# hiroyasuakada/EgoRear

Measured on AMD Instinct MI355X. Metric: 4-view frames/sec (heatmap+MVFEx+3D lift), higher is better.
Workload: dtype f32 (fp16x2 split, 22-bit operands, fp32 accumulate)

## Files before the change

### egorear_amd/csrc/egr_stem_pool.h

```cpp
#pragma once
#include "egr_common.h"

template <int NW>
struct StemPool {
    f32x2 P0[8];
    f32x2 P1[8];
    f32x2 e0, e1;
    float amx = 0.f;

    static __device__ __forceinline__ int pc(int q, int half) { return (q & 1) + 4 * (q >> 1) + 2 * half; }

    __device__ __forceinline__ void reduce(const f32x16 (&acc)[2][2], const float (&sc)[2], const float (&sh)[2], int half) {
#pragma unroll
        for (int j = 0; j < 2; ++j) {
            float vm[16], v1[16];
#pragma unroll
            for (int r = 0; r < 16; ++r) {
                float t0 = acc[0][j][r] * sc[j] + sh[j], t1 = acc[1][j][r] * sc[j] + sh[j];
                t0 = t0 > 0.f ? t0 : 0.f;
                t1 = t1 > 0.f ? t1 : 0.f;
                v1[r] = t1;
                vm[r] = fmaxf(t0, t1);
                amx = fmaxf(amx, vm[r]);
            }
            float om[4], o1[4];
#pragma unroll
            for (int g = 0; g < 4; ++g) { om[g] = __shfl_xor(vm[4 * g + 3], 32); o1[g] = __shfl_xor(v1[4 * g + 3], 32); }
#pragma unroll
            for (int q = 0; q < 8; ++q) {
                const int g = q >> 1;
                float x0 = fmaxf(vm[2 * q], vm[2 * q + 1]), x1 = fmaxf(v1[2 * q], v1[2 * q + 1]);
                if (q & 1) { x0 = fmaxf(x0, vm[2 * q - 1]); x1 = fmaxf(x1, v1[2 * q - 1]); }
                else {
                    const float lm = half ? om[g] : (g > 0 ? om[g - 1] : 0.f), l1 = half ? o1[g] : (g > 0 ? o1[g - 1] : 0.f);
                    x0 = fmaxf(x0, lm); x1 = fmaxf(x1, l1);
                }
                P0[q][j] = x0; P1[q][j] = x1;
            }
            e0[j] = vm[15]; e1[j] = v1[15];
        }
    }

    static constexpr int XFLOATS = (NW - 1) * 16 * 64;

    __device__ __forceinline__ void publish(float* s_x, int wave, int l31, int half) const {
        if (wave < NW - 1) {
#pragma unroll
            for (int q = 0; q < 8; ++q) *reinterpret_cast<f32x2*>(&s_x[(wave * 16 + pc(q, half)) * 64 + 2 * l31]) = P1[q];
        }
    }

    static __device__ __forceinline__ void amax2(float* p, f32x2 v) {
        atomicMax(reinterpret_cast<int*>(p), __float_as_int(v[0]));
        atomicMax(reinterpret_cast<int*>(p) + 1, __float_as_int(v[1]));
    }

    __device__ __forceinline__ void finish(const float* s_x, int wave, int l31, int half, float* y, int n, int oy0, int ox0, int pho, int pwo) {
        if (wave > 0) {
#pragma unroll
            for (int q = 0; q < 8; ++q) {
                const f32x2 u = *reinterpret_cast<const f32x2*>(&s_x[((wave - 1) * 16 + pc(q, half)) * 64 + 2 * l31]);
                P0[q][0] = fmaxf(P0[q][0], u[0]); P0[q][1] = fmaxf(P0[q][1], u[1]);
            }
        }
        const int gp = (oy0 >> 1) + wave, gc0 = ox0 >> 1;
        float* const yrow = y + (((int64_t)n * pho + gp) * pwo + gc0) * 64 + 2 * l31;
        const bool arow = wave == 0 && oy0 > 0;
#pragma unroll
        for (int q = 0; q < 8; ++q) {
            float* const p = yrow + pc(q, half) * 64;
            if (arow || (q == 0 && half == 0 && ox0 > 0)) amax2(p, P0[q]);
            else *reinterpret_cast<f32x2*>(p) = P0[q];
        }
        if (half && gc0 + 16 < pwo) {
            amax2(yrow + 16 * 64, e0);
            if (gp + 1 < pho) amax2(yrow + (int64_t)pwo * 64 + 16 * 64, e1);
        }
        if (wave == NW - 1 && gp + 1 < pho) {
#pragma unroll
            for (int q = 0; q < 8; ++q) amax2(yrow + (int64_t)pwo * 64 + pc(q, half) * 64, P1[q]);
        }
    }
};

template <int NW>
__global__ __launch_bounds__(256) void stem_pool_init_kernel(float* y, int images, int pho, int pwo) {
    const int rows = pho / NW - ((pho % NW) ? 0 : 1), cols = pwo / 16 - ((pwo % 16) ? 0 : 1);
    const int64_t na = (int64_t)images * rows * pwo * 16, nb = (int64_t)images * pho * cols * 16;
    int64_t i = (int64_t)blockIdx.x * 256 + threadIdx.x;
    int n, p, c;
    if (i < na) {
        const int q = (int)(i & 15);
        int64_t t = i >> 4;
        c = (int)(t % pwo); t /= pwo;
        p = ((int)(t % rows) + 1) * NW; n = (int)(t / rows);
        i = q;
    } else if (i < na + nb) {
        i -= na;
        const int q = (int)(i & 15);
        int64_t t = i >> 4;
        c = ((int)(t % cols) + 1) * 16; t /= cols;
        p = (int)(t % pho); n = (int)(t / pho);
        i = q;
    } else return;
    const f32x4 z = {0.f, 0.f, 0.f, 0.f};
    *reinterpret_cast<f32x4*>(y + (((int64_t)n * pho + p) * pwo + c) * 64 + i * 4) = z;
}

template <int NW>
static inline void stem_pool_init(float* y, int64_t images, int pho, int pwo, hipStream_t s) {
    const int rows = pho / NW - ((pho % NW) ? 0 : 1), cols = pwo / 16 - ((pwo % 16) ? 0 : 1);
    const int64_t total = images * ((int64_t)rows * pwo + (int64_t)pho * cols) * 16;
    if (total <= 0) return;
    hipLaunchKernelGGL(stem_pool_init_kernel<NW>, dim3((unsigned)((total + 255) / 256)), dim3(256), 0, s, y, (int)images, pho, pwo);
}
```

### egorear_amd/csrc/egr_stem_x6.hip

```cpp
#include "egr_common.h"
#include "egr_stem_pool.h"

namespace {

typedef __bf16 bf16x8 __attribute__((ext_vector_type(8)));
typedef _Float16 f16x8 __attribute__((ext_vector_type(8)));
typedef unsigned u32x4 __attribute__((ext_vector_type(4)));

constexpr int NW = 8, NT = NW * 64;
constexpr int TH = 2 * NW, TW = 32;
constexpr int PH = 2 * TH + 5;
constexpr int PW = 2 * TW + 5;
constexpr int PWS = 72;
constexpr int PATCH = 3 * PH * PWS;
constexpr int PLOADS = (PATCH + NT - 1) / NT;
constexpr int PPAIRS = (PATCH / 2 + NT - 1) / NT;
static_assert(PATCH % 2 == 0 && PWS % 2 == 0, "pixel pairs");
#ifndef STEM_PRESPLIT
#define STEM_PRESPLIT 1
#endif
#ifndef STEM_KS
#define STEM_KS 11
#endif
constexpr int KS = STEM_KS;
constexpr int WBYTES = KS * 2 * 3 * 1024;
constexpr int WBYTES2 = KS * 2 * 2 * 1024;

static_assert(StemPool<NW>::XFLOATS <= PATCH, "the pooling exchange area lives in a dead patch buffer");

__device__ __forceinline__ unsigned cvt_pk_bf16(float lo, float hi) {
    unsigned r;
    asm("v_cvt_pk_bf16_f32 %0, %1, %2" : "=v"(r) : "v"(lo), "v"(hi));
    return r;
}
__device__ __forceinline__ float bf16_hi_f32(unsigned p) { return __uint_as_float(p & 0xffff0000u); }
__device__ __forceinline__ float bf16_lo_f32(unsigned p) { return __uint_as_float(p << 16); }
__device__ __forceinline__ void split2_f16(float v0, float v1, float s, unsigned& h, unsigned& l) {
    asm("v_fma_mixlo_f16 %0, %1, %2, 0" : "=v"(h) : "v"(v0), "v"(s));
    asm("v_fma_mixhi_f16 %0, %1, %2, 0" : "+v"(h) : "v"(v1), "v"(s));
    asm("v_fma_mixlo_f16 %0, %1, %2, -%3 op_sel_hi:[0,0,1]" : "=v"(l) : "v"(v0), "v"(s), "v"(h));
    asm("v_fma_mixhi_f16 %0, %1, %2, -%3 op_sel:[0,0,1] op_sel_hi:[0,0,1]" : "+v"(l) : "v"(v1), "v"(s), "v"(h));
}
__device__ __forceinline__ void pow2_prescale(unsigned bits, float& s, float& inv) {
    int k = 141 - (int)(bits >> 23);
    k = k > 60 ? 60 : (k < -60 ? -60 : k);
    s = __uint_as_float((unsigned)(127 + k) << 23);
    inv = __uint_as_float((unsigned)(127 - k) << 23);
}

struct StemX6Args {
    const float* x;
    egr_nmap xmap;
    int n, h, w, ho, wo;
    const uint8_t* w6;
    const float* wds;
    const float* scale;
    const float* shift;
    float* y;
    int tiles_x, tiles_y;
    int64_t gx;
    unsigned* amax_out;
};

template <int PH_>
__device__ __forceinline__ constexpr int pair_off_t(int p) {
    const int pp = p > 20 ? 20 : p;
    return (pp / 7) * PH_ * PWS + (pp % 7) * PWS;
}

template <bool POOL, int NPL>
__global__ __launch_bounds__(NT, 1) void stem_x6_kernel(const StemX6Args a) {
    auto pair_off = [](int p) constexpr { return pair_off_t<PH>(p); };
    constexpr int WB = NPL == 3 ? WBYTES : WBYTES2, NPR = NPL == 3 ? 6 : 3;
    constexpr bool PRE = NPL == 2 && STEM_PRESPLIT;
    __shared__ __attribute__((aligned(16))) float s_patch[2][PATCH];
    __shared__ __attribute__((aligned(16))) uint8_t s_w[WB];
    __shared__ unsigned s_pmax[2][NW];
    const int tid = threadIdx.x, lane = tid & 63, wave = tid >> 6;
    const int l31 = lane & 31, half = lane >> 5;
    const int grp = blockIdx.y;
    const int tpi = a.tiles_x * a.tiles_y;
    const int total = a.n * tpi;
    const float* xg = a.x + grp * a.gx;
    const bool raw = a.scale == nullptr;
    float* y = a.y + (int64_t)grp * a.n * (POOL ? (a.ho >> 1) * (a.wo >> 1) : a.ho * a.wo) * 64;

    int p_lds[PLOADS], p_ci[PLOADS], p_py[PLOADS], p_px[PLOADS];
#pragma unroll
    for (int u = 0; u < PLOADS; ++u) {
        const int i = tid + NT * u;
        const int ci = i / (PH * PWS);
        const int r = i - ci * PH * PWS;
        p_ci[u] = ci; p_py[u] = r / PWS; p_px[u] = r - p_py[u] * PWS;
        p_lds[u] = (i < PATCH) ? i : -1;
    }
    auto fetch = [&](int tile, float (&v)[PLOADS]) {
        const int n = tile / tpi;
        const int t = tile - n * tpi;
        const int ty = t / a.tiles_x, tx = t - ty * a.tiles_x;
        const int iy0 = 2 * ty * TH - 3, ix0 = 2 * tx * TW - 3;
        const float* img = xg + egr_map(a.xmap, n);
#pragma unroll
        for (int u = 0; u < PLOADS; ++u) {
            const int iy = iy0 + p_py[u], ix = ix0 + p_px[u];
            const bool ok = p_lds[u] >= 0 && p_px[u] < PW && iy >= 0 && iy < a.h && ix >= 0 && ix < a.w;
            v[u] = ok ? img[((int64_t)p_ci[u] * a.h + iy) * a.w + ix] : 0.f;
        }
    };
    auto park = [&](int buf, const float (&v)[PLOADS]) {
        float m = 0.f;
#pragma unroll
        for (int u = 0; u < PLOADS; ++u)
            if (p_lds[u] >= 0) {
                s_patch[buf][p_lds[u]] = v[u];
                m = fmaxf(m, fabsf(v[u]));
            }
        if constexpr (NPL == 2) {
            m = wave_max(m);
            if (lane == 0) s_pmax[buf][wave] = __float_as_uint(m);
        }
    };
    int q_geo[PRE ? PPAIRS : 1];
    if constexpr (PRE) {
#pragma unroll
        for (int u = 0; u < PPAIRS; ++u) {
            const int i = 2 * (tid + NT * u);
            const int ci = i / (PH * PWS);
            const int r = i - ci * PH * PWS;
            const int py = r / PWS;
            q_geo[u] = (i < PATCH) ? ((ci << 16) | (py << 8) | (r - py * PWS)) : -1;
        }
    }
    auto fetch2 = [&](int tile, float (&v)[2 * PPAIRS]) {
        const int n = tile / tpi;
        const int t = tile - n * tpi;
        const int ty = t / a.tiles_x, tx = t - ty * a.tiles_x;
        const int iy0 = 2 * ty * TH - 3, ix0 = 2 * tx * TW - 3;
        const float* img = xg + egr_map(a.xmap, n);
#pragma unroll
        for (int u = 0; u < (PRE ? PPAIRS : 1); ++u) {
            const int g = q_geo[u], q_ci = g >> 16, q_py = (g >> 8) & 255, q_px = g & 255;
            const int iy = iy0 + q_py, ix = ix0 + q_px;
            const bool rowok = g >= 0 && iy >= 0 && iy < a.h;
            const float* rp = img + ((int64_t)q_ci * a.h + iy) * a.w + ix;
            v[2 * u] = (rowok && q_px < PW && ix >= 0 && ix < a.w) ? rp[0] : 0.f;
            v[2 * u + 1] = (rowok && q_px + 1 < PW && ix + 1 >= 0 && ix + 1 < a.w) ? rp[1] : 0.f;
        }
    };
    auto publish_max = [&](int buf, const float (&v)[2 * PPAIRS]) {
        float m = 0.f;
#pragma unroll
        for (int u = 0; u < 2 * PPAIRS; ++u) m = fmaxf(m, fabsf(v[u]));
        m = wave_max(m);
        if (lane == 0) s_pmax[buf][wave] = __float_as_uint(m);
    };
    auto park2 = [&](int buf, const float (&v)[2 * PPAIRS], float psc_) {
        unsigned* const ph = reinterpret_cast<unsigned*>(s_patch[buf]);
#pragma unroll
        for (int u = 0; u < (PRE ? PPAIRS : 1); ++u)
            if (q_geo[u] >= 0) {
                unsigned h, l;
                split2_f16(v[2 * u], v[2 * u + 1], psc_, h, l);
                ph[tid + NT * u] = h;
                ph[PATCH / 2 + tid + NT * u] = l;
            }
    };
    auto patch_scale = [&](int buf, float& s, float& inv) {
        unsigned m = s_pmax[buf][lane & (NW - 1)];
#pragma unroll
        for (int o = NW / 2; o > 0; o >>= 1) {
            const unsigned other = (unsigned)__shfl_xor((int)m, o, 64);
            m = other > m ? other : m;
        }
        pow2_prescale(__builtin_amdgcn_readfirstlane(m), s, inv);
    };

    {
        const u32x4* src = reinterpret_cast<const u32x4*>(a.w6 + (int64_t)grp * WB);
        for (int i = tid; i < WB / 16; i += NT) reinterpret_cast<u32x4*>(s_w)[i] = src[i];
    }
    float pv[PRE ? 1 : PLOADS];
    float pv2[PRE ? 2 * PPAIRS : 1];
    float psc = 1.f, pinv = 1.f;
    int tile = blockIdx.x;
    if constexpr (PRE) {
        if (tile < total) {
            fetch2(tile, pv2);
            publish_max(0, pv2);
        }
        __syncthreads();
        if (tile < total) {
            patch_scale(0, psc, pinv);
            park2(0, pv2, psc);
        }
    } else {
        if (tile < total) {
            fetch(tile, pv);
            park(0, pv);
        }
    }
    __syncthreads();

    const int abase0 = (2 * (2 * wave)) * PWS + 2 * l31;
    const int abase1 = (2 * (2 * wave + 1)) * PWS + 2 * l31;
    float sc[2], sh[2];
#pragma unroll
    for (int j = 0; j < 2; ++j) {
        sc[j] = raw ? 1.f : a.scale[grp * 64 + 2 * l31 + j];
        sh[j] = raw ? 0.f : a.shift[grp * 64 + 2 * l31 + j];
    }
    float wds[2] = {1.f, 1.f};
    if constexpr (NPL == 2) {
        wds[0] = a.wds[grp * 64 + 2 * l31];
        wds[1] = a.wds[grp * 64 + 2 * l31 + 1];
    }

    int buf = 0;
    float amx = 0.f;
    for (; tile < total; tile += gridDim.x, buf ^= 1) {
        const int next = tile + gridDim.x;
        if (next < total) {
            if constexpr (PRE) fetch2(next, pv2);
            else fetch(next, pv);
        }
        const float* sp = s_patch[buf];
        if constexpr (NPL == 2 && !PRE) patch_scale(buf, psc, pinv);
        const float pinv_cur = pinv;
        f32x16 acc[2][2];
#pragma unroll
        for (int i = 0; i < 2; ++i)
#pragma unroll
            for (int j = 0; j < 2; ++j)
#pragma unroll
                for (int r = 0; r < 16; ++r) acc[i][j][r] = 0.f;

        f32x2 raw_a[2][4];
        u32x4 sa[2][2][NPL];
        u32x4 bfr[2][2][NPL];
        auto read_a_pre = [&](int s, int par) {
            const int ao = half ? pair_off(2 * s + 1) : pair_off(2 * s);
            const unsigned* const ph = reinterpret_cast<const unsigned*>(sp);
            const unsigned* h0 = ph + ((abase0 + ao) >> 1);
            const unsigned* h1 = ph + ((abase1 + ao) >> 1);
#pragma unroll
            for (int e = 0; e < 4; ++e) {
                sa[par][0][0][e] = h0[e];
                sa[par][0][1][e] = h0[PATCH / 2 + e];
                sa[par][1][0][e] = h1[e];
                sa[par][1][1][e] = h1[PATCH / 2 + e];
            }
        };
        auto read_a = [&](int s) {
            const int ao = half ? pair_off(2 * s + 1) : pair_off(2 * s);
            const float* q0 = sp + abase0 + ao;
            const float* q1 = sp + abase1 + ao;
#pragma unroll
            for (int e = 0; e < 4; ++e) {
                raw_a[0][e] = *reinterpret_cast<const f32x2*>(q0 + 2 * e);
                raw_a[1][e] = *reinterpret_cast<const f32x2*>(q1 + 2 * e);
            }
        };
        auto read_b = [&](int s, int par) {
#pragma unroll
            for (int j = 0; j < 2; ++j)
#pragma unroll
                for (int pl = 0; pl < NPL; ++pl)
                    bfr[par][j][pl] = *reinterpret_cast<const u32x4*>(s_w + ((s * 2 + j) * NPL + pl) * 1024 + lane * 16);
        };
        auto split_pair = [&](int par, int i, int e) {
            const float v0 = raw_a[i][e][0], v1 = raw_a[i][e][1];
            if constexpr (NPL == 3) {
                const unsigned h = cvt_pk_bf16(v0, v1);
                const float r0 = v0 - bf16_lo_f32(h), r1 = v1 - bf16_hi_f32(h);
                const unsigned m = cvt_pk_bf16(r0, r1);
                sa[par][i][0][e] = h;
                sa[par][i][1][e] = m;
                sa[par][i][2][e] = cvt_pk_bf16(r0 - bf16_lo_f32(m), r1 - bf16_hi_f32(m));
            } else {
                unsigned h, l;
                split2_f16(v0, v1, psc, h, l);
                sa[par][i][0][e] = h;
                sa[par][i][1][e] = l;
            }
        };
        if constexpr (PRE) {
            read_a_pre(0, 0);
        } else {
            read_a(0);
        }
        read_b(0, 0);
        if constexpr (!PRE) {
#pragma unroll
            for (int c = 0; c < 8; ++c) split_pair(0, c >> 2, c & 3);
        }
#pragma unroll
        for (int s = 0; s < KS; ++s) {
            const int par = s & 1;
            if (s + 1 < KS) {
                if constexpr (PRE) read_a_pre(s + 1, par ^ 1);
                else read_a(s + 1);
                read_b(s + 1, par ^ 1);
            }
            __builtin_amdgcn_sched_barrier(0);
            constexpr int PA[6] = {NPL == 3 ? 2 : 1, 0, NPL == 3 ? 1 : 0, 1, 0, 0}, PB[6] = {0, NPL == 3 ? 2 : 1, NPL == 3 ? 1 : 0, 0, 1, 0};
            constexpr int EVERY = NPL == 3 ? 3 : 1;
            int nm = 0;
#pragma unroll
            for (int t = 0; t < NPR; ++t)
#pragma unroll
                for (int i = 0; i < 2; ++i)
#pragma unroll
                    for (int j = 0; j < 2; ++j, ++nm) {
                        if constexpr (NPL == 3)
                            acc[i][j] = __builtin_amdgcn_mfma_f32_32x32x16_bf16(__builtin_bit_cast(bf16x8, sa[par][i][PA[t]]),
                                                                                __builtin_bit_cast(bf16x8, bfr[par][j][PB[t]]), acc[i][j], 0, 0, 0);
                        else
                            acc[i][j] = __builtin_amdgcn_mfma_f32_32x32x16_f16(__builtin_bit_cast(f16x8, sa[par][i][PA[t]]),
                                                                               __builtin_bit_cast(f16x8, bfr[par][j][PB[t]]), acc[i][j], 0, 0, 0);
                        if (!PRE && s + 1 < KS && nm % EVERY == EVERY - 1 && nm / EVERY < 8) {
                            const int c = nm / EVERY;
                            split_pair(par ^ 1, c >> 2, c & 3);
                            __builtin_amdgcn_sched_barrier(0);
                        }
                    }
        }
        if constexpr (NPL == 2) {
#pragma unroll
            for (int i = 0; i < 2; ++i)
#pragma unroll
                for (int j = 0; j < 2; ++j) {
                    const float dsc = pinv_cur * wds[j];
#pragma unroll
                    for (int r = 0; r < 16; ++r) acc[i][j][r] *= dsc;
                }
        }

        const int n = tile / tpi;
        const int t = tile - n * tpi;
        const int ty = t / a.tiles_x, tx = t - ty * a.tiles_x;
        const int oy0 = ty * TH, ox0 = tx * TW;
#ifdef STEM_SKIP_EPI
        if (acc[0][0][0] + acc[0][1][1] + acc[1][0][2] + acc[1][1][3] == 12345.f) y[tid] = 1.f;
        if constexpr (PRE) {
            if (next < total) publish_max(buf ^ 1, pv2);
            __syncthreads();
            if (next < total) { patch_scale(buf ^ 1, psc, pinv); park2(buf ^ 1, pv2, psc); }
        } else {
            if (next < total) park(buf ^ 1, pv);
        }
        __syncthreads();
        continue;
#endif
        if constexpr (POOL) {
            StemPool<NW> pool;
            pool.reduce(acc, sc, sh, half);
            if constexpr (PRE) {
                if (next < total) publish_max(buf ^ 1, pv2);
            }
            __syncthreads();
            pool.publish(s_patch[buf], wave, l31, half);
            if constexpr (PRE) {
                if (next < total) { patch_scale(buf ^ 1, psc, pinv); park2(buf ^ 1, pv2, psc); }
            } else {
                if (next < total) park(buf ^ 1, pv);
            }
            __syncthreads();
            pool.finish(s_patch[buf], wave, l31, half, y, n, oy0, ox0, a.ho >> 1, a.wo >> 1);
            amx = fmaxf(amx, pool.amx);
        } else {
#pragma unroll
            for (int i = 0; i < 2; ++i) {
                const int oy = oy0 + 2 * wave + i;
#pragma unroll
                for (int r = 0; r < 16; ++r) {
                    const int ox = ox0 + (r & 3) + 8 * (r >> 2) + 4 * half;
                    f32x2 v;
                    v[0] = acc[i][0][r] * sc[0] + sh[0];
                    v[1] = acc[i][1][r] * sc[1] + sh[1];
                    if (!raw) {
                        v[0] = v[0] > 0.f ? v[0] : 0.f;
                        v[1] = v[1] > 0.f ? v[1] : 0.f;
                    }
                    *reinterpret_cast<f32x2*>(&y[(((int64_t)n * a.ho + oy) * a.wo + ox) * 64 + 2 * l31]) = v;
                }
            }
            if constexpr (PRE) {
                if (next < total) publish_max(buf ^ 1, pv2);
                __syncthreads();
                if (next < total) { patch_scale(buf ^ 1, psc, pinv); park2(buf ^ 1, pv2, psc); }
            } else {
                if (next < total) park(buf ^ 1, pv);
            }
            __syncthreads();
        }
    }
    if (POOL && a.amax_out) {
        amx = wave_max(amx);
        if (lane == 0 && amx > 0.f)
            __hip_atomic_fetch_max(a.amax_out + ((blockIdx.x * NW + wave) & 63), __float_as_uint(amx), __ATOMIC_RELAXED, __HIP_MEMORY_SCOPE_AGENT);
    }
}

__global__ __launch_bounds__(64) void pack_stem_w6_kernel(const float* __restrict__ w, uint8_t* __restrict__ img) {
    const int lane = threadIdx.x, j = blockIdx.x & 1, s = blockIdx.x >> 1, grp = blockIdx.y;
    const int co = 2 * (lane & 31) + j, p = 2 * s + (lane >> 5);
    const float* wr = w + ((int64_t)grp * 64 + co) * 148;
    u32x4 h, m, l;
#pragma unroll
    for (int e = 0; e < 4; ++e) {
        float v[2];
#pragma unroll
        for (int z = 0; z < 2; ++z) {
            const int kw = 2 * e + z;
            v[z] = (p <= 20 && kw < 7) ? wr[p * 7 + kw] : 0.f;
        }
        h[e] = cvt_pk_bf16(v[0], v[1]);
        const float r0 = v[0] - bf16_lo_f32(h[e]), r1 = v[1] - bf16_hi_f32(h[e]);
        m[e] = cvt_pk_bf16(r0, r1);
        l[e] = cvt_pk_bf16(r0 - bf16_lo_f32(m[e]), r1 - bf16_hi_f32(m[e]));
    }
    uint8_t* dst = img + (int64_t)grp * WBYTES + ((s * 2 + j) * 3) * 1024 + lane * 16;
    *reinterpret_cast<u32x4*>(dst) = h;
    *reinterpret_cast<u32x4*>(dst + 1024) = m;
    *reinterpret_cast<u32x4*>(dst + 2048) = l;
}

__global__ __launch_bounds__(64) void pack_stem_wh2_kernel(const float* __restrict__ w, uint8_t* __restrict__ img, float* __restrict__ descale) {
    const int lane = threadIdx.x, j = blockIdx.x & 1, s = blockIdx.x >> 1, grp = blockIdx.y;
    const int co = 2 * (lane & 31) + j, p = 2 * s + (lane >> 5);
    const float* wr = w + ((int64_t)grp * 64 + co) * 148;
    float m = 0.f;
    for (int k = 0; k < 147; ++k) m = fmaxf(m, fabsf(wr[k]));
    float sc, inv;
    pow2_prescale(__float_as_uint(m), sc, inv);
    if (s == 0 && lane < 32) descale[grp * 64 + co] = inv;
    u32x4 h, l;
#pragma unroll
    for (int e = 0; e < 4; ++e) {
        float v[2];
#pragma unroll
        for (int z = 0; z < 2; ++z) {
            const int kw = 2 * e + z;
            v[z] = (p <= 20 && kw < 7) ? wr[p * 7 + kw] : 0.f;
        }
        unsigned hh, ll;
        split2_f16(v[0], v[1], sc, hh, ll);
        h[e] = hh;
        l[e] = ll;
    }
    uint8_t* dst = img + (int64_t)grp * WBYTES2 + ((s * 2 + j) * 2) * 1024 + lane * 16;
    *reinterpret_cast<u32x4*>(dst) = h;
    *reinterpret_cast<u32x4*>(dst + 1024) = l;
}

}

extern "C" int64_t egr_stem_wh2_bytes(void) { return WBYTES2; }

extern "C" int egr_pack_stem_wh2_f32(const float* w, int32_t groups, void* img, float* descale, void* stream) {
    if (!w || !img || !descale) return EGR_ENULL;
    if (groups <= 0 || groups > 65535 || ((uintptr_t)img & 15)) return EGR_EINVAL;
    hipLaunchKernelGGL(pack_stem_wh2_kernel, dim3(KS * 2, (unsigned)groups), dim3(64), 0, (hipStream_t)stream, w, (uint8_t*)img, descale);
    return egr_launch_status();
}

extern "C" int64_t egr_stem_w6_bytes(void) { return WBYTES; }

extern "C" int egr_pack_stem_w6_f32(const float* w, int32_t groups, void* img, void* stream) {
    if (!w || !img) return EGR_ENULL;
    if (groups <= 0 || groups > 65535 || ((uintptr_t)img & 15)) return EGR_EINVAL;
    hipLaunchKernelGGL(pack_stem_w6_kernel, dim3(KS * 2, (unsigned)groups), dim3(64), 0, (hipStream_t)stream, w, (uint8_t*)img);
    return egr_launch_status();
}

static int stem_x6_run(const float* x, egr_nmap xmap, int32_t n, int32_t h, int32_t w, const void* w6, const float* scale, const float* shift,
                       float* y, int32_t pool, int32_t groups, int64_t gx, uint32_t* amax_out, void* stream, const float* wds = nullptr);

extern "C" int egr_stem_conv7x7_h2_f32(const float* x, egr_nmap xmap, int32_t n, int32_t h, int32_t w, const void* wh2, const float* w_descale,
                                       const float* scale, const float* shift, float* y, int32_t pool, int32_t groups, int64_t gx,
                                       uint32_t* amax_out, void* stream) {
    if (!w_descale) return EGR_ENULL;
    if (amax_out && !pool) return EGR_EINVAL;
    return stem_x6_run(x, xmap, n, h, w, wh2, scale, shift, y, pool, groups, gx, amax_out, stream, w_descale);
}

extern "C" int egr_stem_conv7x7_x6_f32(const float* x, egr_nmap xmap, int32_t n, int32_t h, int32_t w, const void* w6,
                                       const float* scale, const float* shift, float* y, int32_t pool, int32_t groups, int64_t gx,
                                       void* stream) {
    return stem_x6_run(x, xmap, n, h, w, w6, scale, shift, y, pool, groups, gx, nullptr, stream);
}

extern "C" int egr_stem_conv7x7_x6_ex_f32(const float* x, egr_nmap xmap, int32_t n, int32_t h, int32_t w, const void* w6,
                                          const float* scale, const float* shift, float* y, int32_t pool, int32_t groups, int64_t gx,
                                          uint32_t* amax_out, void* stream) {
    if (amax_out && !pool) return EGR_EINVAL;
    return stem_x6_run(x, xmap, n, h, w, w6, scale, shift, y, pool, groups, gx, amax_out, stream);
}

static int stem_x6_run(const float* x, egr_nmap xmap, int32_t n, int32_t h, int32_t w, const void* w6, const float* scale, const float* shift,
                       float* y, int32_t pool, int32_t groups, int64_t gx, uint32_t* amax_out, void* stream, const float* wds) {
    if (!x || !w6 || !y || ((scale == nullptr) != (shift == nullptr))) return EGR_ENULL;
    if (pool && !scale) return EGR_EINVAL;
    if (groups <= 0 || groups > 65535 || ((uintptr_t)w6 & 15)) return EGR_EINVAL;
    if (n <= 0 || h <= 0 || w <= 0 || h % (2 * TH) != 0 || w % (2 * TW) != 0 || xmap.n_inner <= 0) return EGR_EINVAL;
    StemX6Args a;
    a.x = x; a.xmap = xmap; a.n = n; a.h = h; a.w = w; a.ho = h / 2; a.wo = w / 2;
    a.w6 = (const uint8_t*)w6; a.scale = scale; a.shift = shift; a.y = y;
    a.tiles_x = a.wo / TW; a.tiles_y = a.ho / TH;
    a.gx = gx;
    a.amax_out = amax_out;
    a.wds = wds;
    const int64_t tiles = (int64_t)n * a.tiles_x * a.tiles_y;
    if (tiles >= (1LL << 31)) return EGR_EINVAL;
    int64_t blocks = 256 / groups;
    if (blocks < 1) blocks = 1;
    if (blocks > tiles) blocks = tiles;
    hipStream_t s = (hipStream_t)stream;
    if (pool) {
        stem_pool_init<NW>(y, (int64_t)groups * n, a.ho / 2, a.wo / 2, s);
        if (wds) hipLaunchKernelGGL((stem_x6_kernel<true, 2>), dim3((unsigned)blocks, (unsigned)groups), dim3(NT), 0, s, a);
        else hipLaunchKernelGGL((stem_x6_kernel<true, 3>), dim3((unsigned)blocks, (unsigned)groups), dim3(NT), 0, s, a);
    } else {
        if (wds) hipLaunchKernelGGL((stem_x6_kernel<false, 2>), dim3((unsigned)blocks, (unsigned)groups), dim3(NT), 0, s, a);
        else hipLaunchKernelGGL((stem_x6_kernel<false, 3>), dim3((unsigned)blocks, (unsigned)groups), dim3(NT), 0, s, a);
    }
    return egr_launch_status();
}
```

Baseline: 6741.

## Vectorize stem patch loads into 16-byte units with lane-shuffle alignment fixup

The presplit stem patch fetch now loads four floats per lane with a single unaligned vector load. A ds_bpermute pulls the neighbour's first element so the unit lines up with the patch columns, and interior tiles skip per-element bounds checks. Tile coordinates advance incrementally instead of being recomputed with divisions, the per-element dequant multiply folds into the epilogue scale, and the pool amax is taken on the pooled values. This cuts global load instructions and VALU work, but adds cross-lane permutes, always-issued loads, and edge-case logic that could break correctness.

Result: no change. 6792, median of 6 (+0.7%).

```diff
diff --git a/egorear_amd/csrc/egr_stem_pool.h b/egorear_amd/csrc/egr_stem_pool.h
--- a/egorear_amd/csrc/egr_stem_pool.h
+++ b/egorear_amd/csrc/egr_stem_pool.h
@@ -21,7 +21,6 @@
                 t1 = t1 > 0.f ? t1 : 0.f;
                 v1[r] = t1;
                 vm[r] = fmaxf(t0, t1);
-                amx = fmaxf(amx, vm[r]);
             }
             float om[4], o1[4];
 #pragma unroll
@@ -36,6 +35,7 @@
                     x0 = fmaxf(x0, lm); x1 = fmaxf(x1, l1);
                 }
                 P0[q][j] = x0; P1[q][j] = x1;
+                amx = fmaxf(amx, x0);
             }
             e0[j] = vm[15]; e1[j] = v1[15];
         }
@@ -64,21 +64,23 @@
             }
         }
         const int gp = (oy0 >> 1) + wave, gc0 = ox0 >> 1;
-        float* const yrow = y + (((int64_t)n * pho + gp) * pwo + gc0) * 64 + 2 * l31;
+        float* const yrow = y + (((int64_t)n * pho + gp) * pwo + gc0) * 64;
+        float* const ynext = yrow + (int64_t)pwo * 64;
+        const unsigned lo = 128u * half + 2u * l31;
         const bool arow = wave == 0 && oy0 > 0;
 #pragma unroll
         for (int q = 0; q < 8; ++q) {
-            float* const p = yrow + pc(q, half) * 64;
+            float* const p = yrow + (lo + pc(q, 0) * 64u);
             if (arow || (q == 0 && half == 0 && ox0 > 0)) amax2(p, P0[q]);
             else *reinterpret_cast<f32x2*>(p) = P0[q];
         }
         if (half && gc0 + 16 < pwo) {
-            amax2(yrow + 16 * 64, e0);
-            if (gp + 1 < pho) amax2(yrow + (int64_t)pwo * 64 + 16 * 64, e1);
+            amax2(yrow + (lo + 14u * 64u), e0);
+            if (gp + 1 < pho) amax2(ynext + (lo + 14u * 64u), e1);
         }
         if (wave == NW - 1 && gp + 1 < pho) {
 #pragma unroll
-            for (int q = 0; q < 8; ++q) amax2(yrow + (int64_t)pwo * 64 + pc(q, half) * 64, P1[q]);
+            for (int q = 0; q < 8; ++q) amax2(ynext + (lo + pc(q, 0) * 64u), P1[q]);
         }
     }
 };
diff --git a/egorear_amd/csrc/egr_stem_x6.hip b/egorear_amd/csrc/egr_stem_x6.hip
--- a/egorear_amd/csrc/egr_stem_x6.hip
+++ b/egorear_amd/csrc/egr_stem_x6.hip
@@ -6,6 +6,7 @@
 typedef __bf16 bf16x8 __attribute__((ext_vector_type(8)));
 typedef _Float16 f16x8 __attribute__((ext_vector_type(8)));
 typedef unsigned u32x4 __attribute__((ext_vector_type(4)));
+typedef unsigned u32x2 __attribute__((ext_vector_type(2)));
 
 constexpr int NW = 8, NT = NW * 64;
 constexpr int TH = 2 * NW, TW = 32;
@@ -14,8 +15,13 @@
 constexpr int PWS = 72;
 constexpr int PATCH = 3 * PH * PWS;
 constexpr int PLOADS = (PATCH + NT - 1) / NT;
-constexpr int PPAIRS = (PATCH / 2 + NT - 1) / NT;
 static_assert(PATCH % 2 == 0 && PWS % 2 == 0, "pixel pairs");
+constexpr int PU = PWS / 4;
+constexpr int NUNITS = 3 * PH * PU;
+constexpr int ULOADS = (NUNITS + 63 * NW - 1) / (63 * NW);
+static_assert(PWS % 4 == 0 && PW + 1 <= PWS && 4 * (PU - 1) < PW, "a row's last unit keeps patch column 4 PU - 4 and is zero from PW on");
+static_assert((PATCH / 2) % 2 == 0, "8-byte aligned plane l");
+typedef float f32x4u __attribute__((ext_vector_type(4), aligned(4)));
 #ifndef STEM_PRESPLIT
 #define STEM_PRESPLIT 1
 #endif
@@ -76,11 +82,31 @@
     __shared__ __attribute__((aligned(16))) float s_patch[2][PATCH];
     __shared__ __attribute__((aligned(16))) uint8_t s_w[WB];
     __shared__ unsigned s_pmax[2][NW];
-    const int tid = threadIdx.x, lane = tid & 63, wave = tid >> 6;
+    const int tid = threadIdx.x, lane = tid & 63, wave = __builtin_amdgcn_readfirstlane(tid >> 6);
     const int l31 = lane & 31, half = lane >> 5;
     const int grp = blockIdx.y;
     const int tpi = a.tiles_x * a.tiles_y;
     const int total = a.n * tpi;
+    struct Pos { int n, ty, tx; };
+    const int st_n = (int)gridDim.x / tpi, st_r = (int)gridDim.x - st_n * tpi, st_y = st_r / a.tiles_x, st_x = st_r - st_y * a.tiles_x;
+    auto advance = [&](Pos p) {
+        p.tx += st_x;
+        const int cx = p.tx >= a.tiles_x;
+        p.tx -= cx ? a.tiles_x : 0;
+        p.ty += st_y + cx;
+        const int cy = p.ty >= a.tiles_y;
+        p.ty -= cy ? a.tiles_y : 0;
+        p.n += st_n + cy;
+        return p;
+    };
+    Pos pos;
+    {
+        const int t0 = (int)blockIdx.x;
+        pos.n = t0 / tpi;
+        const int t = t0 - pos.n * tpi;
+        pos.ty = t / a.tiles_x;
+        pos.tx = t - pos.ty * a.tiles_x;
+    }
     const float* xg = a.x + grp * a.gx;
     const bool raw = a.scale == nullptr;
     float* y = a.y + (int64_t)grp * a.n * (POOL ? (a.ho >> 1) * (a.wo >> 1) : a.ho * a.wo) * 64;
@@ -94,10 +120,8 @@
         p_ci[u] = ci; p_py[u] = r / PWS; p_px[u] = r - p_py[u] * PWS;
         p_lds[u] = (i < PATCH) ? i : -1;
     }
-    auto fetch = [&](int tile, float (&v)[PLOADS]) {
-        const int n = tile / tpi;
-        const int t = tile - n * tpi;
-        const int ty = t / a.tiles_x, tx = t - ty * a.tiles_x;
+    auto fetch = [&](const Pos& tp, float (&v)[PLOADS]) {
+        const int n = tp.n, ty = tp.ty, tx = tp.tx;
         const int iy0 = 2 * ty * TH - 3, ix0 = 2 * tx * TW - 3;
         const float* img = xg + egr_map(a.xmap, n);
 #pragma unroll
@@ -120,49 +144,72 @@
             if (lane == 0) s_pmax[buf][wave] = __float_as_uint(m);
         }
     };
-    int q_geo[PRE ? PPAIRS : 1];
+    unsigned u_off[PRE ? ULOADS : 1];
+    int u_geo[PRE ? ULOADS : 1];
+    const int nb_addr = ((lane + 1) & 63) * 4;
     if constexpr (PRE) {
 #pragma unroll
-        for (int u = 0; u < PPAIRS; ++u) {
-            const int i = 2 * (tid + NT * u);
-            const int ci = i / (PH * PWS);
-            const int r = i - ci * PH * PWS;
-            const int py = r / PWS;
-            q_geo[u] = (i < PATCH) ? ((ci << 16) | (py << 8) | (r - py * PWS)) : -1;
-        }
-    }
-    auto fetch2 = [&](int tile, float (&v)[2 * PPAIRS]) {
-        const int n = tile / tpi;
-        const int t = tile - n * tpi;
-        const int ty = t / a.tiles_x, tx = t - ty * a.tiles_x;
-        const int iy0 = 2 * ty * TH - 3, ix0 = 2 * tx * TW - 3;
-        const float* img = xg + egr_map(a.xmap, n);
-#pragma unroll
-        for (int u = 0; u < (PRE ? PPAIRS : 1); ++u) {
-            const int g = q_geo[u], q_ci = g >> 16, q_py = (g >> 8) & 255, q_px = g & 255;
-            const int iy = iy0 + q_py, ix = ix0 + q_px;
-            const bool rowok = g >= 0 && iy >= 0 && iy < a.h;
-            const float* rp = img + ((int64_t)q_ci * a.h + iy) * a.w + ix;
-            v[2 * u] = (rowok && q_px < PW && ix >= 0 && ix < a.w) ? rp[0] : 0.f;
-            v[2 * u + 1] = (rowok && q_px + 1 < PW && ix + 1 >= 0 && ix + 1 < a.w) ? rp[1] : 0.f;
-        }
-    };
-    auto publish_max = [&](int buf, const float (&v)[2 * PPAIRS]) {
+        for (int u = 0; u < ULOADS; ++u) {
+            const int i = 63 * (NW * u + wave) + lane;
+            const int ii = i < NUNITS ? i : 0;
+            const int r = ii / PU, k = ii - r * PU;
+            const int ci = r / PH, py = r - ci * PH;
+            u_off[u] = (unsigned)((ci * a.h + py) * a.w + 4 * k);
+            u_geo[u] = (py << 8) | k | ((i < NUNITS && lane < 63) ? 1 << 16 : 0) | (k == PU - 1 ? 1 << 17 : 0);
+        }
+    }
+    auto fetch4 = [&](const Pos& tp, f32x4 (&q)[PRE ? ULOADS : 1], unsigned& ok) {
+        const int iy0 = 2 * tp.ty * TH - 3, ix0 = 2 * tp.tx * TW - 4;
+        const float* img = xg + egr_map(a.xmap, tp.n);
+        const int worg = iy0 * a.w + ix0;
+        const bool interior = tp.tx > 0 && tp.tx + 1 < a.tiles_x && tp.ty > 0 && tp.ty + 1 < a.tiles_y;
+        unsigned off[PRE ? ULOADS : 1];
+        ok = (1u << ULOADS) - 1;
+        if (interior) {
+#pragma unroll
+            for (int u = 0; u < (PRE ? ULOADS : 1); ++u) off[u] = u_off[u] + (unsigned)worg;
+        } else {
+#pragma unroll
+            for (int u = 0; u < (PRE ? ULOADS : 1); ++u) {
+                const int iy = iy0 + ((u_geo[u] >> 8) & 255), ix = ix0 + 4 * (u_geo[u] & 255);
+                const bool in = iy >= 0 && iy < a.h && ix >= 0 && ix < a.w;
+                off[u] = in ? u_off[u] + (unsigned)worg : 0u;
+                ok &= in ? ~0u : ~(1u << u);
+            }
+        }
+#pragma unroll
+        for (int u = 0; u < (PRE ? ULOADS : 1); ++u) q[u] = *reinterpret_cast<const f32x4u*>(img + off[u]);
+    };
+    auto publish_max = [&](int buf, f32x4 (&q)[PRE ? ULOADS : 1], unsigned ok) {
         float m = 0.f;
 #pragma unroll
-        for (int u = 0; u < 2 * PPAIRS; ++u) m = fmaxf(m, fabsf(v[u]));
+        for (int u = 0; u < (PRE ? ULOADS : 1); ++u) {
+            const bool in = (ok >> u) & 1, body = in && !((u_geo[u] >> 17) & 1);
+            const float q0 = in ? q[u][0] : 0.f;
+            const float nb = __int_as_float(__builtin_amdgcn_ds_bpermute(nb_addr, __float_as_int(q0)));
+            f32x4 v;
+            v[0] = in ? q[u][1] : 0.f;
+            v[1] = body ? q[u][2] : 0.f;
+            v[2] = body ? q[u][3] : 0.f;
+            v[3] = (u_geo[u] >> 17) & 1 ? 0.f : nb;
+            q[u] = v;
+            m = fmaxf(fmaxf(m, fmaxf(fabsf(v[0]), fabsf(v[1]))), fmaxf(fabsf(v[2]), fabsf(v[3])));
+        }
         m = wave_max(m);
         if (lane == 0) s_pmax[buf][wave] = __float_as_uint(m);
     };
-    auto park2 = [&](int buf, const float (&v)[2 * PPAIRS], float psc_) {
-        unsigned* const ph = reinterpret_cast<unsigned*>(s_patch[buf]);
-#pragma unroll
-        for (int u = 0; u < (PRE ? PPAIRS : 1); ++u)
-            if (q_geo[u] >= 0) {
-                unsigned h, l;
-                split2_f16(v[2 * u], v[2 * u + 1], psc_, h, l);
-                ph[tid + NT * u] = h;
-                ph[PATCH / 2 + tid + NT * u] = l;
+    auto park4 = [&](int buf, const f32x4 (&q)[PRE ? ULOADS : 1], float psc_) {
+        u32x2* const ph = reinterpret_cast<u32x2*>(s_patch[buf]);
+#pragma unroll
+        for (int u = 0; u < (PRE ? ULOADS : 1); ++u)
+            if ((u_geo[u] >> 16) & 1) {
+                unsigned h0, l0, h1, l1;
+                split2_f16(q[u][0], q[u][1], psc_, h0, l0);
+                split2_f16(q[u][2], q[u][3], psc_, h1, l1);
+                const u32x2 h = {h0, h1}, l = {l0, l1};
+                const int i = 63 * (NW * u + wave) + lane;
+                ph[i] = h;
+                ph[PATCH / 4 + i] = l;
             }
     };
     auto patch_scale = [&](int buf, float& s, float& inv) {
@@ -180,22 +227,23 @@
         for (int i = tid; i < WB / 16; i += NT) reinterpret_cast<u32x4*>(s_w)[i] = src[i];
     }
     float pv[PRE ? 1 : PLOADS];
-    float pv2[PRE ? 2 * PPAIRS : 1];
+    f32x4 pv2[PRE ? ULOADS : 1];
+    unsigned pok = 0;
     float psc = 1.f, pinv = 1.f;
     int tile = blockIdx.x;
     if constexpr (PRE) {
         if (tile < total) {
-            fetch2(tile, pv2);
-            publish_max(0, pv2);
+            fetch4(pos, pv2, pok);
+            publish_max(0, pv2, pok);
         }
         __syncthreads();
         if (tile < total) {
             patch_scale(0, psc, pinv);
-            park2(0, pv2, psc);
+            park4(0, pv2, psc);
         }
     } else {
         if (tile < total) {
-            fetch(tile, pv);
+            fetch(pos, pv);
             park(0, pv);
         }
     }
@@ -209,20 +257,20 @@
         sc[j] = raw ? 1.f : a.scale[grp * 64 + 2 * l31 + j];
         sh[j] = raw ? 0.f : a.shift[grp * 64 + 2 * l31 + j];
     }
-    float wds[2] = {1.f, 1.f};
+    float scw[2] = {sc[0], sc[1]};
     if constexpr (NPL == 2) {
-        wds[0] = a.wds[grp * 64 + 2 * l31];
-        wds[1] = a.wds[grp * 64 + 2 * l31 + 1];
+        scw[0] *= a.wds[grp * 64 + 2 * l31];
+        scw[1] *= a.wds[grp * 64 + 2 * l31 + 1];
     }
 
     int buf = 0;
     float amx = 0.f;
     for (; tile < total; tile += gridDim.x, buf ^= 1) {
         const int next = tile + gridDim.x;
-        if (next < total) {
-            if constexpr (PRE) fetch2(next, pv2);
-            else fetch(next, pv);
-        }
+        const Pos cur = pos;
+        pos = advance(pos);
+        if constexpr (PRE) fetch4(next < total ? pos : cur, pv2, pok);
+        else if (next < total) fetch(pos, pv);
         const float* sp = s_patch[buf];
         if constexpr (NPL == 2 && !PRE) patch_scale(buf, psc, pinv);
         const float pinv_cur = pinv;
@@ -324,27 +372,20 @@
                         }
                     }
         }
+        float sct[2] = {scw[0], scw[1]};
         if constexpr (NPL == 2) {
-#pragma unroll
-            for (int i = 0; i < 2; ++i)
-#pragma unroll
-                for (int j = 0; j < 2; ++j) {
-                    const float dsc = pinv_cur * wds[j];
-#pragma unroll
-                    for (int r = 0; r < 16; ++r) acc[i][j][r] *= dsc;
-                }
-        }
-
-        const int n = tile / tpi;
-        const int t = tile - n * tpi;
-        const int ty = t / a.tiles_x, tx = t - ty * a.tiles_x;
-        const int oy0 = ty * TH, ox0 = tx * TW;
+            sct[0] *= pinv_cur;
+            sct[1] *= pinv_cur;
+        }
+
+        const int n = cur.n;
+        const int oy0 = cur.ty * TH, ox0 = cur.tx * TW;
 #ifdef STEM_SKIP_EPI
         if (acc[0][0][0] + acc[0][1][1] + acc[1][0][2] + acc[1][1][3] == 12345.f) y[tid] = 1.f;
         if constexpr (PRE) {
-            if (next < total) publish_max(buf ^ 1, pv2);
+            publish_max(buf ^ 1, pv2, pok);
             __syncthreads();
-            if (next < total) { patch_scale(buf ^ 1, psc, pinv); park2(buf ^ 1, pv2, psc); }
+            if (next < total) { patch_scale(buf ^ 1, psc, pinv); park4(buf ^ 1, pv2, psc); }
         } else {
             if (next < total) park(buf ^ 1, pv);
         }
@@ -353,14 +394,14 @@
 #endif
         if constexpr (POOL) {
             StemPool<NW> pool;
-            pool.reduce(acc, sc, sh, half);
+            pool.reduce(acc, sct, sh, half);
             if constexpr (PRE) {
-                if (next < total) publish_max(buf ^ 1, pv2);
+                publish_max(buf ^ 1, pv2, pok);
             }
             __syncthreads();
             pool.publish(s_patch[buf], wave, l31, half);
             if constexpr (PRE) {
-                if (next < total) { patch_scale(buf ^ 1, psc, pinv); park2(buf ^ 1, pv2, psc); }
+                if (next < total) { patch_scale(buf ^ 1, psc, pinv); park4(buf ^ 1, pv2, psc); }
             } else {
                 if (next < total) park(buf ^ 1, pv);
             }
@@ -375,8 +416,8 @@
                 for (int r = 0; r < 16; ++r) {
                     const int ox = ox0 + (r & 3) + 8 * (r >> 2) + 4 * half;
                     f32x2 v;
-                    v[0] = acc[i][0][r] * sc[0] + sh[0];
-                    v[1] = acc[i][1][r] * sc[1] + sh[1];
+                    v[0] = acc[i][0][r] * sct[0] + sh[0];
+                    v[1] = acc[i][1][r] * sct[1] + sh[1];
                     if (!raw) {
                         v[0] = v[0] > 0.f ? v[0] : 0.f;
                         v[1] = v[1] > 0.f ? v[1] : 0.f;
@@ -385,9 +426,9 @@
                 }
             }
             if constexpr (PRE) {
-                if (next < total) publish_max(buf ^ 1, pv2);
+                publish_max(buf ^ 1, pv2, pok);
                 __syncthreads();
-                if (next < total) { patch_scale(buf ^ 1, psc, pinv); park2(buf ^ 1, pv2, psc); }
+                if (next < total) { patch_scale(buf ^ 1, psc, pinv); park4(buf ^ 1, pv2, psc); }
             } else {
                 if (next < total) park(buf ^ 1, pv);
             }
@@ -511,7 +552,7 @@
     a.amax_out = amax_out;
     a.wds = wds;
     const int64_t tiles = (int64_t)n * a.tiles_x * a.tiles_y;
-    if (tiles >= (1LL << 31)) return EGR_EINVAL;
+    if (tiles >= (1LL << 31) || (int64_t)3 * h * w >= (1LL << 31)) return EGR_EINVAL;
     int64_t blocks = 256 / groups;
     if (blocks < 1) blocks = 1;
     if (blocks > tiles) blocks = tiles;
```
